# Wenlin-Chen/ADKF-IFT

Measured on AMD Instinct MI355X. Metric: meta-tasks/sec (N_support=128, d=256), higher is better.
Workload: dtype f32

## Files before the change

### adkf_ift_amd/_lib.py

```python
from __future__ import annotations

import ctypes as C
import os

_HERE = os.path.dirname(os.path.abspath(__file__))
LIB_PATH = os.path.join(_HERE, "libadkf_gp.so")
if os.environ.get("ADKF_LIB"):
    LIB_PATH = os.environ["ADKF_LIB"]

KERNEL_RBF = 0
KERNEL_MATERN52 = 1
IGNORE_GRAD_CORRECTION = 1
IGNORE_DIRECT_GRAD = 2
INFO_OUTER_BASE = 100000
PM_LATENT = 1
PM_MAXIMIZE = 2
PM_SCORE_MEAN = 4
POOL_TOPK_MAX = 64
TS_SAMPLES_MAX = 64
TS_FEATURES_MAX = 4096

ERRORS = {-1: "bad argument", -2: "unsupported size (see adkf_max_points)", -3: "workspace too small",
          -4: "HIP launch failed"}


class Batch(C.Structure):
    _fields_ = [("T", C.c_int32), ("ns_max", C.c_int32), ("nq_max", C.c_int32), ("d", C.c_int32),
                ("kernel", C.c_int32), ("flags", C.c_int32),
                ("n_s", C.c_void_p), ("n_q", C.c_void_p), ("Z_s", C.c_void_p), ("y_s", C.c_void_p),
                ("Z_q", C.c_void_p), ("y_q", C.c_void_p), ("priors", C.c_void_p)]


class MsgEt(C.Structure):
    _fields_ = [("src", C.c_void_p), ("tgt", C.c_void_p), ("W", C.c_void_p), ("bias", C.c_void_p), ("dW", C.c_void_p),
                ("db", C.c_void_p), ("E", C.c_int32)]


class FitOptions(C.Structure):
    _fields_ = [("max_evals", C.c_int32), ("exact_evals", C.c_int32), ("gtol", C.c_float), ("ftol", C.c_float),
                ("ev_start", C.c_void_p), ("ev_stop", C.c_void_p)]


_lib = None

SIGNATURES = {
    "adkf_version": (C.c_char_p, []),
    "adkf_last_hip_error": (C.c_char_p, []),
    "adkf_max_points": (C.c_int, []),
    "adkf_path_info": (C.c_int, [C.c_int32, C.c_int32]),
    "adkf_workspace_bytes": (C.c_size_t, [C.c_int32] * 4),
    "adkf_median_lengthscale": (C.c_int, [C.POINTER(Batch), C.c_void_p, C.c_void_p, C.c_size_t, C.c_void_p]),
    "adkf_init_params": (C.c_int, [C.POINTER(Batch), C.c_int32, C.c_int32, C.c_void_p, C.c_void_p, C.c_void_p,
                                   C.c_void_p, C.c_size_t, C.c_void_p]),
    "adkf_mll_value_grad": (C.c_int, [C.POINTER(Batch), C.c_void_p, C.c_void_p, C.c_void_p, C.c_void_p, C.c_void_p,
                                      C.c_void_p, C.c_size_t, C.c_void_p]),
    "adkf_fit": (C.c_int, [C.POINTER(Batch), C.c_void_p, C.POINTER(FitOptions), C.c_void_p, C.c_void_p, C.c_void_p,
                           C.c_void_p, C.c_void_p, C.c_size_t, C.c_void_p]),
    "adkf_predict": (C.c_int, [C.POINTER(Batch), C.c_void_p, C.c_void_p, C.c_void_p, C.c_void_p, C.c_void_p,
                               C.c_void_p, C.c_size_t, C.c_void_p]),
    "adkf_predict_marginal": (C.c_int, [C.POINTER(Batch), C.c_void_p, C.c_int32, C.c_void_p, C.c_void_p, C.c_int64, C.c_void_p,
                                        C.c_void_p, C.c_void_p, C.c_void_p, C.c_void_p, C.c_void_p, C.c_size_t, C.c_void_p]),
    "adkf_predict_marginal_ard": (C.c_int, [C.POINTER(Batch), C.c_void_p, C.c_int32, C.c_void_p, C.c_void_p, C.c_int64, C.c_void_p,
                                            C.c_void_p, C.c_void_p, C.c_void_p, C.c_void_p, C.c_void_p, C.c_size_t, C.c_void_p]),
    "adkf_predict_pool_scratch_bytes": (C.c_size_t, [C.c_int32, C.c_int32]),
    "adkf_predict_pool": (C.c_int, [C.POINTER(Batch), C.c_void_p, C.c_int32, C.c_void_p, C.c_int64, C.c_void_p, C.c_void_p, C.c_void_p,
                                    C.c_void_p, C.c_void_p, C.c_void_p, C.c_int32, C.c_void_p, C.c_void_p, C.c_void_p, C.c_void_p,
                                    C.c_size_t, C.c_void_p, C.c_size_t, C.c_void_p]),
    "adkf_thompson_pool_scratch_bytes": (C.c_size_t, [C.c_int32] * 4),
    "adkf_thompson_pool": (C.c_int, [C.POINTER(Batch), C.c_void_p, C.c_int32, C.c_void_p, C.c_int64, C.c_void_p, C.c_void_p, C.c_int32,
                                     C.c_void_p, C.c_void_p, C.c_int32, C.c_void_p, C.c_void_p, C.c_void_p, C.c_void_p, C.c_void_p,
                                     C.c_void_p, C.c_void_p, C.c_size_t, C.c_void_p, C.c_size_t, C.c_void_p]),
    "adkf_thompson_pool_ard": (C.c_int, [C.POINTER(Batch), C.c_void_p, C.c_int32, C.c_void_p, C.c_int64, C.c_void_p, C.c_void_p, C.c_int32,
                                         C.c_void_p, C.c_void_p, C.c_int32, C.c_void_p, C.c_void_p, C.c_void_p, C.c_void_p, C.c_void_p,
                                         C.c_void_p, C.c_void_p, C.c_size_t, C.c_void_p, C.c_size_t, C.c_void_p]),
    "adkf_outer_nll_value_grad": (C.c_int, [C.POINTER(Batch), C.c_void_p, C.c_void_p, C.c_void_p, C.c_void_p,
                                            C.c_void_p, C.c_void_p, C.c_void_p, C.c_size_t, C.c_void_p]),
    "adkf_ift_hypergrad": (C.c_int, [C.POINTER(Batch), C.c_void_p, C.c_int32, C.c_void_p, C.c_void_p, C.c_void_p,
                                     C.c_void_p, C.c_void_p, C.c_void_p, C.c_void_p, C.c_void_p, C.c_size_t,
                                     C.c_void_p]),
    "adkf_check_info": (C.c_int, [C.c_void_p, C.c_int32, C.c_void_p]),
    "adkf_workspace_bytes_ard": (C.c_size_t, [C.c_int32] * 4),
    "adkf_msg_forward": (C.c_int, [C.c_void_p, C.c_void_p, C.c_int32, C.c_int32, C.c_int32, C.c_int32, C.c_void_p, C.c_void_p]),
# ... 61 lines not shown
```

### adkf_ift_amd/csrc/adkf_gp.hip

```cpp
#include <hip/hip_runtime.h>
#include <algorithm>
#include <cstdio>
#include <cstdlib>

#include "../../include/adkf_gp.h"
#include "ard.h"
#include "pna.h"
#include "readout.h"
#include "block.h"
#include "outer_step.h"
#include "refine64.h"
#include "hyper.h"
#include "large_fused.h"
#include "gemm_x3.h"
#include "dense_x3.h"
#include "predict_stream.h"
#include "thompson_stream.h"

using namespace adkf;

namespace {

constexpr int MAX_POINTS = 4096;
constexpr int REG_POINTS = 128;

inline size_t align_up(size_t x) { return (x + 255) & ~size_t(255); }

inline int grid_for(int T, int tiles) { return ((T + 7) / 8) * 8 * tiles; }
inline int ceil_div(int a, int b) { return (a + b - 1) / b; }

inline int tiles_of(int M, int N) { return ceil_div(M, GT) * ceil_div(N, GT); }

template <class P> struct use_x3 : std::false_type {};
template <> struct use_x3<ProbDistMulti> : std::true_type {};
bool x3_enabled() {
    static const bool v = [] { const char* e = getenv("ADKF_X3"); return !(e && e[0] == '0'); }();
    return v;
}

inline bool x3_for(int d) { return x3_enabled() && d >= GK; }

template <class P>
void launch_gemm(const P& p, int T, int M, int N, hipStream_t st, bool x3 = false) {
    const int tm = ceil_div(M, GT), tn = ceil_div(N, GT);
    if constexpr (use_x3<P>::value) {
        if (x3 && x3_enabled()) { k_bgemm3<P, GT, 256><<<((T + 7) / 8) * 8 * tm * tn, 256, 0, st>>>(p, T, tm, tn); return; }
    }
    k_bgemm<P, GT><<<((T + 7) / 8) * 8 * tm * tn, 256, 0, st>>>(p, T, tm, tn);
}

// ... 370 lines not shown
        k_lg_resid<<<dim3(ceil_div(nq, 4), a.T), 256, 0, st>>>(a);
        LgMat m = lg_mat(w, a.S, a.tv.nq_ld, a.tv.n_q, nullptr, a.T);
        lg_sweep(m, st);
        LgMatvecArgs mv{m, a.vecs + (size_t)V_R * a.tv.vld, (size_t)NVEC * a.tv.vld, a.vecs + (size_t)V_E * a.tv.vld, (size_t)NVEC * a.tv.vld, -1.f};
        k_lg_matvec<<<dim3(ceil_div(nq, 4), a.T), 256, 0, st>>>(mv);
        const int tn = ceil_div(nq, GT);
        k_lg_negate<<<grid_for(a.T, tn * tn), 256, 0, st>>>(m, tn);
        LgColsumArgs cs{a.C, a.tv.ns_ld, (size_t)a.tv.nq_ld * a.tv.ns_ld, a.tv.n_q, a.tv.nq_ld, a.tv.n_s, a.tv.ns_ld,
                        a.vecs + (size_t)V_E * a.tv.vld, (size_t)NVEC * a.tv.vld, a.vecs + (size_t)V_CTE * a.tv.vld, (size_t)NVEC * a.tv.vld};
        k_lg_colsum<<<dim3(ceil_div(a.tv.ns_ld, 64), a.T), 1024, 0, st>>>(cs);
        LgOuterFin fin{a, w.lg_logdet, w.lg_info, w.lg_pext};
        k_lg_outer_fin<<<a.T, 64, 0, st>>>(fin);
        LAUNCH_OK();
        return 0;
    }
    if (nq <= 16) k_outer_factor<16, 256><<<grid_for(a.T, 1), 256, 0, st>>>(a);
    else if (nq <= 32) k_outer_factor<32, 256><<<grid_for(a.T, 1), 256, 0, st>>>(a);
    else if (nq <= 64) k_outer_factor<64, 256><<<grid_for(a.T, 1), 256, 0, st>>>(a);
    else k_outer_factor<128, 512><<<grid_for(a.T, 1), 512, 0, st>>>(a);
    LAUNCH_OK();
    return 0;
}


InnerArgs inner_args(const adkf_batch_t* b, const Workspace& w, float* phi, int32_t* info) {
    InnerArgs a{};
    a.D2ss = w.D2ss; a.y_s = b->y_s; a.n_s = b->n_s; a.phi = phi; a.priors = b->priors;
    a.Ainv = w.Ainv; a.vecs = w.vecs; a.scal = w.scal; a.info = info;
    a.T = b->T; a.ld = b->ns_max; a.vld = w.vld; a.kind = b->kernel;
    a.max_evals = 0; a.exact_evals = 0; a.gtol = 0.f; a.ftol = 0.f;
    return a;
}

int outer_pipeline(const adkf_batch_t* b, const Workspace& w, const float* phi, int flags, bool with_hessian, float* f_out,
                   float* dZ_s, float* dZ_q, float* g_phi_out, float* v_out, float* H_out, int32_t* info, hipStream_t st) {
    const int T = b->T, ns = b->ns_max, nq = b->nq_max, d = b->d;
    int rc = stage_dist(b, w, true, st);
    if (rc) return rc;
    const bool reuse_inner = (b->flags & ADKF_BATCH_REUSE_INNER) != 0;
    if (!reuse_inner) {
        InnerArgs ia = inner_args(b, w, const_cast<float*>(phi), info);
        rc = launch_inner(ia, w, st);
        if (rc) return rc;
    }
    TaskView tv = make_tv(b, w, true);
    const int tms = ceil_div(ns, GT), tmq = ceil_div(nq, GT);
    const float dirscale = (flags & ADKF_IGNORE_DIRECT_GRAD) ? 0.f : 1.f;
    const float corrscale = (with_hessian && !(flags & ADKF_IGNORE_GRAD_CORRECTION)) ? 1.f : 0.f;
    if (use_fused_outer(ns, nq)) {
        HyperArgs ha{tv, w.Ainv, w.D2ss, w.D2qs, w.D2qq, b->y_s, b->y_q, b->priors, w.Wss, w.Wqs, w.Wqq, w.P, w.OC, w.S, w.vecs, w.scal, f_out, info,
                     g_phi_out, v_out, H_out, T, reuse_inner ? 1 : 0, with_hessian ? 1 : 0, flags, dirscale, corrscale, refine32_threshold()};
        const bool full = ns == HY_N && nq == HY_N && !b->n_s && !b->n_q && tv.vec;
        const bool rbf = b->kernel == ADKF_KERNEL_RBF;
        if (full && rbf) k_hyper<true, 0><<<grid_for(T, 1), HY_NT, HY_LDS_BYTES, st>>>(ha);
        else if (full) k_hyper<true, 1><<<grid_for(T, 1), HY_NT, HY_LDS_BYTES, st>>>(ha);
        else if (rbf) k_hyper<false, 0><<<grid_for(T, 1), HY_NT, HY_LDS_BYTES, st>>>(ha);
        else k_hyper<false, 1><<<grid_for(T, 1), HY_NT, HY_LDS_BYTES, st>>>(ha);
    } else {
    launch_alpha_refine(tv, b, w, st);
    if (with_hessian) {
        ProbP pp; pp.tv = tv; pp.Ainv = w.Ainv; pp.D2ss = w.D2ss; pp.P = w.P;
        launch_gemm(pp, T, ns, ns, st);
        HessArgs ha{tv, w.Ainv, w.P, w.D2ss, b->y_s, b->priors, w.scal, w.vecs, T};
        if (ns > REG_POINTS) {
            k_lg_hess_mv<<<dim3(ceil_div(ns, 4), T), 256, 0, st>>>(ha);
            LgMat am = lg_mat(w, w.Ainv, ns, b->n_s, nullptr, T);
// ... 5 lines not shown
        } else {
            k_hess<<<grid_for(T, 1), SMALL_NT, 0, st>>>(ha);
        }
    }
    launch_c(tv, b, w, st);
    ProbS ps; ps.tv = tv; ps.C = w.C; ps.D2qs = w.D2qs; ps.D2qq = w.D2qq; ps.S = w.S;
    launch_gemm(ps, T, nq, nq, st);
    OuterArgs oa{tv, w.C, w.S, b->y_s, b->y_q, w.vecs, w.scal, f_out, info, T, reuse_inner ? 1 : 0};
    rc = launch_outer_factor(oa, w, nq, st);
    if (rc) return rc;
    ProbOC po; po.tv = tv; po.Sinv = w.S; po.C = w.C; po.D2qs = w.D2qs; po.OC = w.OC; po.Wqs = w.Wqs; po.part = w.part_oc; po.ntiles = w.nt_oc; po.dirscale = dirscale;
    launch_gemm(po, T, nq, ns, st);
    ProbMA pm; pm.tv = tv; pm.C = w.C; pm.OC = w.OC; pm.D2ss = w.D2ss; pm.Wss = w.Wss; pm.part = w.part_ma; pm.ntiles = w.nt_ma; pm.dirscale = dirscale;
    launch_gemm(pm, T, ns, ns, st);
    SolveArgs sa{tv, w.scal, w.vecs, w.part_oc, w.part_ma, w.nt_oc, w.nt_ma, flags, g_phi_out, v_out, H_out, T, with_hessian ? 1 : 0};
    WqqArgs wq{tv, w.S, w.D2qq, w.Wqq, w.scal, dirscale, T, 0, sa};
    if (nq > REG_POINTS) {
        LgWqq lw{wq, w.lg_part, tmq * tmq, tmq};
        k_lg_wqq<<<grid_for(T, tmq * tmq), 256, 0, st>>>(lw);
        k_lg_wqq_fin<<<T, 64, 0, st>>>(lw);
        k_solve_v<<<T, 64, 0, st>>>(sa);
    } else {
        wq.do_solve = 1;
        k_wqq<<<grid_for(T, 1), SMALL_NT, 0, st>>>(wq);
    }
    if (corrscale != 0.f) {
        ProbMixed px; px.tv = tv; px.Ainv = w.Ainv; px.P = w.P; px.D2ss = w.D2ss; px.Wss = w.Wss; px.corrscale = corrscale;
        launch_gemm(px, T, ns, ns, st);
    }
    }
    if (dZ_s || dZ_q) {
        if (dZ_s && b->n_s) hipMemsetAsync(dZ_s, 0, (size_t)T * ns * d * sizeof(float), st);
        if (dZ_q && b->n_q) hipMemsetAsync(dZ_q, 0, (size_t)T * nq * d * sizeof(float), st);
        ProbDZ<false> pzs; pzs.tv = tv; pzs.Wss = w.Wss; pzs.Wqs = w.Wqs; pzs.Wqq = w.Wqq; pzs.Zs = b->Z_s; pzs.Zq = b->Z_q; pzs.dZ = dZ_s; pzs.d = d;
        ProbDZ<true> pzq; pzq.tv = tv; pzq.Wss = w.Wss; pzq.Wqs = w.Wqs; pzq.Wqq = w.Wqq; pzq.Zs = b->Z_s; pzq.Zq = b->Z_q; pzq.dZ = dZ_q; pzq.d = d;
        if (dZ_s) launch_gemm(pzs, T, ns, d, st, x3_for(d));
        if (dZ_q) launch_gemm(pzq, T, nq, d, st, x3_for(d));
    }
    if (w.w64) {
        size_t lds_bytes;
        const Refine64Args ra = refine_args(tv, b, w, with_hessian, 2, f_out, info, nullptr, nullptr, nullptr, lds_bytes);
        Cot64Args ca{tv, b->Z_s, b->Z_q, dZ_s, dZ_q, d, w.vecs, w.scal, w.w64, w.w64_stride, r64_threshold(), T,
                     with_hessian ? 1 : 0, flags, dirscale, corrscale, g_phi_out, v_out, H_out, lds_bytes ? 1 : 0};
        k_tail64<<<T, R64_NT, lds_bytes, st>>>(ra, ca);
    }
    LAUNCH_OK();
    return 0;
}


struct ArdWs {
    float *mu, *ell, *Zt_s, *Zt_q, *G, *Gd_s, *Gd_q, *Gdot, *phi3, *pri3, *f3, *g3, *g3o, *S1, *gt, *coldot;
    float *c, *ut2, *wn, *Ddot, *Wdot, *adot, *S2;
    ArdFitState* fst; float *x, *g, *p, *xe, *ge, *S, *Y, *fe; int32_t* info3;
    ArdCgState* cst; float *cx, *cr, *cp, *cHp, *gout; int32_t* n_eff;
    size_t bytes;
};

ArdWs carve_ard(void* base, size_t off0, int T, int ns, int nq, int d) {
    ArdWs a;
    size_t off = off0;
    auto take = [&](size_t nfloat) { float* p = base ? reinterpret_cast<float*>(static_cast<char*>(base) + off) : nullptr; off += align_up((nfloat ? nfloat : 1) * sizeof(float)); return p; };
    const size_t Tz = (size_t)T, h = 2 + (size_t)d;
    a.mu = take(Tz * d); a.ell = take(Tz * d);
    a.Zt_s = take(Tz * ns * d); a.Zt_q = take(Tz * nq * d);
    a.G = take(Tz * ns * d); a.Gd_s = take(Tz * ns * d); a.Gd_q = take(Tz * nq * d); a.Gdot = take(Tz * ns * d);
    a.phi3 = take(Tz * 3); a.pri3 = take(Tz * 4); a.f3 = take(Tz); a.g3 = take(Tz * 3); a.g3o = take(Tz * 3);
    a.S1 = take(Tz * d); a.gt = take(Tz * h); a.coldot = take(Tz * d);
    a.c = take(Tz * d); a.ut2 = take(Tz * 2); a.wn = take(Tz * ns);
    a.Ddot = take(Tz * ns * ns); a.Wdot = take(Tz * ns * ns); a.adot = take(Tz * ns); a.S2 = take(Tz * d);
// ... 135 lines not shown

int predict_core(const adkf_batch_t* b, const Workspace& w, float* mean, float* var, float* cov, int32_t* info, hipStream_t st) {
    TaskView tv = make_tv(b, w, true);
    const int T = b->T;
    launch_alpha_refine(tv, b, w, st);
    launch_c(tv, b, w, st);
    launch_refine(tv, b, w, false, 1, nullptr, info, st);
    PredArgs pa{tv, w.C, w.D2qs, b->y_s, mean, var, w.scal, T};
    k_predict<<<grid_for(T, 1), 256, 0, st>>>(pa);
    if (cov) {
        hipMemsetAsync(cov, 0, (size_t)T * b->nq_max * b->nq_max * sizeof(float), st);
        ProbS ps; ps.tv = tv; ps.C = w.C; ps.D2qs = w.D2qs; ps.D2qq = w.D2qq; ps.S = cov;
        launch_gemm(ps, T, b->nq_max, b->nq_max, st);
    }
    LAUNCH_OK();
    return 0;
}

int ard_outer(ArdCtx& c, const float* phi, int flags, float* f_out, int32_t* info, bool want_grads) {
    hipStream_t st = c.st;
    int rc;
    if (!(c.b->flags & ADKF_BATCH_REUSE_INNER)) {
        rc = ard_eval(c, phi, c.a.fe, c.a.ge, c.a.info3);
        if (rc) return rc;
        hipMemcpyAsync(info, c.a.info3, sizeof(int32_t) * (size_t)c.T, hipMemcpyDeviceToDevice, st);
    } else {
        hipMemsetAsync(info, 0, sizeof(int32_t) * (size_t)c.T, st);
    }
    k_ard_scale<<<dim3(ceil_div(c.nq, 4), c.T), 256, 0, st>>>(c.v, c.b->Z_q, c.a.Zt_q, c.b->n_q, c.nq);
    rc = stage_dist(&c.bt, c.w, true, st, 2 | 4);
    if (rc) return rc;
    if (!want_grads) return 0;
    adkf_batch_t bq = c.bt;
    bq.flags = ADKF_BATCH_REUSE_DIST | ADKF_BATCH_REUSE_INNER;
    int32_t* info_o = c.a.info3;
    rc = outer_pipeline(&bq, c.w, c.a.phi3, flags & ADKF_IGNORE_DIRECT_GRAD, false, f_out, c.a.Gd_s, c.a.Gd_q, c.a.g3o, nullptr, nullptr, info_o, st);
    if (rc) return rc;
    ArdColdot cd{c.a.Zt_s, c.a.Gd_s, c.b->n_s, c.ns, c.a.Zt_q, c.a.Gd_q, c.b->n_q, c.nq, c.a.coldot, c.d};
    k_ard_coldot<<<dim3(ceil_div(c.d, 64), c.T), 256, 0, st>>>(cd);
    ArdGout go{c.v, phi, c.a.coldot, c.a.g3o, c.a.gout};
    k_ard_gout<<<dim3(ceil_div(c.d, 256), c.T), 256, 0, st>>>(go);
    LAUNCH_OK();
    return 0;
}

__global__ void k_merge_info(const int32_t* extra, int32_t* info, int T) {
    const int t = blockIdx.x * blockDim.x + threadIdx.x;
    if (t < T && info[t] == 0 && extra[t] != 0) info[t] = extra[t];
}

int ard_ift(const adkf_batch_t* b, const float* phi, int flags, bool with_hessian, int cg_maxiter, float cg_tol, float* f_out,
            float* dZ_s, float* dZ_q, float* g_phi_out, float* v_out, int32_t* cg_iters, int32_t* info, void* ws, size_t ws_bytes,
            hipStream_t st) {
    ArdCtx c;
    int rc = ard_setup(b, ws, ws_bytes, st, c);
    if (rc) return rc;
    if (b->flags & ADKF_BATCH_REUSE_INNER) k_ard_params<<<dim3(ceil_div(c.d, 256), c.T), 256, 0, st>>>(c.v, phi);
    rc = ard_outer(c, phi, flags, f_out, info, true);
    if (rc) return rc;
    k_merge_info<<<ceil_div(c.T, 64), 64, 0, st>>>(c.a.info3, info, c.T);
    const size_t hb = sizeof(float) * (size_t)c.T * c.h;
    if (g_phi_out) hipMemcpyAsync(g_phi_out, c.a.gout, hb, hipMemcpyDeviceToDevice, st);
    const bool correct = with_hessian && !(flags & ADKF_IGNORE_GRAD_CORRECTION);
    if (correct) {
        ArdCg cg{c.T, c.h, cg_tol, c.a.cst, c.a.gout, c.a.cx, c.a.cr, c.a.cp, c.a.cHp, b->n_s, c.ns, c.a.n_eff};
        k_ard_cg_begin<<<c.T, 256, 0, st>>>(cg);
        FitPoll poll(true, cg_maxiter, c.a.info3, st);
// ... 532 lines not shown
                           const int64_t* excl_off, float* paths, int64_t* sel_idx, float* sel_val, int32_t* info, void* ws, size_t ws_bytes,
                           void* scratch, size_t scratch_bytes, void* stream) {
    return thompson_pool(true, b, phi, flags, X, rows, omega, phase, m, w, eps, S, excl_idx, excl_off, paths, sel_idx, sel_val, info, ws,
                         ws_bytes, scratch, scratch_bytes, stream);
}

int adkf_outer_nll_value_grad(const adkf_batch_t* b, const float* phi, float* f_out, float* g_phi, float* dZ_s,
                              float* dZ_q, int32_t* info, void* ws, size_t ws_bytes, void* stream) {
    int rc = check_batch(b, true);
    if (rc) return rc;
    if (!phi || !f_out || !info || !ws || !b->y_s || !b->y_q || !b->priors) return ADKF_E_BADARG;
    if (is_ard(b))
        return ard_ift(b, phi, 0, false, 0, 0.f, f_out, dZ_s, dZ_q, g_phi, nullptr, nullptr, info, ws, ws_bytes, static_cast<hipStream_t>(stream));
    Workspace w = carve_for(b, ws);
    if (ws_bytes < w.bytes) return ADKF_E_WORKSPACE;
    return outer_pipeline(b, w, phi, 0, false, f_out, dZ_s, dZ_q, g_phi, nullptr, nullptr, info, static_cast<hipStream_t>(stream));
}

int adkf_ift_hypergrad(const adkf_batch_t* b, const float* phi, int32_t flags, float* f_out, float* dZ_s, float* dZ_q,
                       float* g_phi_out, float* v, float* H, int32_t* info, void* ws, size_t ws_bytes, void* stream) {
    int rc = check_batch(b, true);
    if (rc) return rc;
    if (!phi || !f_out || !dZ_s || !dZ_q || !info || !ws || !b->y_s || !b->y_q || !b->priors) return ADKF_E_BADARG;
    if (is_ard(b)) {
        if (H) return ADKF_E_BADARG;
        return ard_ift(b, phi, flags, true, ADKF_CG_DEFAULT_MAXITER, ADKF_CG_DEFAULT_TOL, f_out, dZ_s, dZ_q, g_phi_out, v, nullptr, info,
                       ws, ws_bytes, static_cast<hipStream_t>(stream));
    }
    Workspace w = carve_for(b, ws);
    if (ws_bytes < w.bytes) return ADKF_E_WORKSPACE;
    return outer_pipeline(b, w, phi, flags, true, f_out, dZ_s, dZ_q, g_phi_out, v, H, info, static_cast<hipStream_t>(stream));
}

int adkf_double_path_tasks(const adkf_batch_t* b, int32_t* flagged, void* ws, size_t ws_bytes, void* stream) {
    int rc = check_batch(b, true);
    if (rc) return rc;
    if (!flagged || !ws || is_ard(b)) return ADKF_E_BADARG;
    Workspace w = carve_for(b, ws);
    if (ws_bytes < w.bytes) return ADKF_E_WORKSPACE;
    (void)hipGetLastError();
    k_double_path_tasks<<<ceil_div(b->T, 256), 256, 0, static_cast<hipStream_t>(stream)>>>(w.scal, b->ns_max, b->nq_max, w.w64 ? r64_threshold() : INFINITY, b->T, flagged);
    LAUNCH_OK();
    return 0;
}

size_t adkf_workspace_bytes_ard(int32_t T, int32_t ns_max, int32_t nq_max, int32_t d) {
    if (T <= 0 || ns_max <= 0 || nq_max < 0 || d <= 0) return 0;
    return carve_ard(nullptr, carve(nullptr, T, ns_max, nq_max, d).bytes, T, ns_max, nq_max, d).bytes;
}

int adkf_ift_hypergrad_cg(const adkf_batch_t* b, const float* phi, int32_t flags, int32_t cg_maxiter, float cg_tol, float* f_out,
                          float* dZ_s, float* dZ_q, float* g_phi_out, float* v, int32_t* cg_iters, int32_t* info, void* ws,
                          size_t ws_bytes, void* stream) {
    int rc = check_batch(b, true);
    if (rc) return rc;
    if (!is_ard(b) || cg_maxiter < 1 || !(cg_tol > 0.f)) return ADKF_E_BADARG;
    if (!phi || !f_out || !dZ_s || !dZ_q || !info || !ws || !b->y_s || !b->y_q || !b->priors) return ADKF_E_BADARG;
    return ard_ift(b, phi, flags, true, cg_maxiter, cg_tol, f_out, dZ_s, dZ_q, g_phi_out, v, cg_iters, info, ws, ws_bytes,
                   static_cast<hipStream_t>(stream));
}

namespace {
long msg_table(MsgArgs& m, const adkf_msg_et_t* ets, int n_et, bool backward) {
    long e_all = 0;
    int splits = 0;
    for (int q = 0; q < n_et; ++q) {
// ... 400 lines not shown
```

### adkf_ift_amd/csrc/cpu/adkf_gp_cpu.cpp

```cpp
#include <algorithm>
#include <cmath>
#include <cstdint>
#include <cstring>
#include <limits>
#include <vector>

#include "adkf_gp.h"

namespace {

using Mat = std::vector<double>;
constexpr double NOISE_LB = 1e-4, LOG_2PI = 1.8378770664093453, SQRT5 = 2.23606797749979;

inline double softplus(double x) { return x > 30.0 ? x : std::log1p(std::exp(x)); }
inline double sigmoid(double x) { return 1.0 / (1.0 + std::exp(-x)); }
inline double inv_softplus(double y) { return y > 30.0 ? y : y + std::log(-std::expm1(-y)); }

inline void kappa(int kind, double u, double& k0, double& k1, double& k2) {
    if (kind == ADKF_KERNEL_RBF) { k0 = std::exp(-0.5 * u); k1 = -0.5 * k0; k2 = 0.25 * k0; return; }
    const double r = std::sqrt(u), e = std::exp(-SQRT5 * r);
    k0 = (1.0 + SQRT5 * r + (5.0 / 3.0) * u) * e; k1 = -(5.0 / 6.0) * (1.0 + SQRT5 * r) * e; k2 = (25.0 / 12.0) * e;
}

template <class F>
// ... 379 lines not shown
    void reset_H() { for (int i = 0; i < 3; ++i) for (int j = 0; j < 3; ++j) Hi[i][j] = i == j; first = true; }
    bool direction() {
        for (int i = 0; i < 3; ++i) p[i] = -(Hi[i][0] * g[0] + Hi[i][1] * g[1] + Hi[i][2] * g[2]);
        gp = g[0] * p[0] + g[1] * p[1] + g[2] * p[2];
        if (!(gp < 0.0)) { reset_H(); for (int i = 0; i < 3; ++i) p[i] = -g[i]; gp = -(g[0] * g[0] + g[1] * g[1] + g[2] * g[2]); if (!(gp < 0.0)) return false; }
        step = first ? std::min(1.0, 1.0 / (std::fabs(g[0]) + std::fabs(g[1]) + std::fabs(g[2]))) : 1.0;
        step = std::min(step, 16.0 / std::max(std::max(std::fabs(p[0]), std::fabs(p[1])), std::max(std::fabs(p[2]), 1e-30)));
        bt = 0;
        return true;
    }
    void accept(const double* xn, double fn, const double* gn) {
        double s[3], yv[3];
        for (int i = 0; i < 3; ++i) { s[i] = xn[i] - x[i]; yv[i] = gn[i] - g[i]; x[i] = xn[i]; g[i] = gn[i]; }
        f = fn;
        const double sy = s[0] * yv[0] + s[1] * yv[1] + s[2] * yv[2], yy = yv[0] * yv[0] + yv[1] * yv[1] + yv[2] * yv[2], ss = s[0] * s[0] + s[1] * s[1] + s[2] * s[2];
        if (sy > 1e-10 * std::sqrt(ss * yy) && yy > 0.0) {
            if (first) { const double sc = sy / yy; for (int i = 0; i < 3; ++i) for (int j = 0; j < 3; ++j) Hi[i][j] = i == j ? sc : 0.0; first = false; }
            const double rho = 1.0 / sy;
            double Hy[3];
            for (int i = 0; i < 3; ++i) Hy[i] = Hi[i][0] * yv[0] + Hi[i][1] * yv[1] + Hi[i][2] * yv[2];
            const double yHy = yv[0] * Hy[0] + yv[1] * Hy[1] + yv[2] * Hy[2];
            for (int i = 0; i < 3; ++i) for (int j = 0; j < 3; ++j) Hi[i][j] += -rho * (s[i] * Hy[j] + Hy[i] * s[j]) + rho * (rho * yHy + 1.0) * s[i] * s[j];
        }
    }
};

}

extern "C" {

const char* adkf_version(void) { return "adkf_gp_cpu 0.1 (float64 inside, OpenMP over tasks)"; }
const char* adkf_last_hip_error(void) { return "no HIP in the CPU twin"; }
int adkf_max_points(void) { return 1 << 20; }
size_t adkf_workspace_bytes(int32_t, int32_t, int32_t, int32_t) { return 0; }

int adkf_median_lengthscale(const adkf_batch_t* b, float* l0, void*, size_t, void*) {
    if (int rc = check(b, false)) return rc;
    if (!l0) return ADKF_E_BADARG;
#pragma omp parallel for schedule(dynamic)
    for (int t = 0; t < b->T; ++t) {
        const int n = ns_of(b, t);
        const float* Z = b->Z_s + (size_t)t * b->ns_max * b->d;
        l0[t] = n > 1 ? (float)median_l0(sqdist(Z, n, Z, n, b->d), n) : 0.f;
    }
    return 0;
}

int adkf_init_params(const adkf_batch_t* b, int32_t numeric, int32_t use_ls_prior, float* phi, float* priors, float* l0, void*, size_t, void*) {
    if (int rc = check(b, false)) return rc;
    if (!phi || !priors) return ADKF_E_BADARG;
#pragma omp parallel for schedule(dynamic)
    for (int t = 0; t < b->T; ++t) {
        const int n = ns_of(b, t);
        const float* Z = b->Z_s + (size_t)t * b->ns_max * b->d;
        const float l = n > 1 ? (float)median_l0(sqdist(Z, n, Z, n, b->d), n) : 0.f;
        if (l0) l0[t] = l;
        const double scale = 0.25, mode = numeric ? 0.01 : 0.1;
        phi[t * 3 + 0] = (float)inv_softplus(mode - NOISE_LB); phi[t * 3 + 1] = 0.f; phi[t * 3 + 2] = (float)inv_softplus((double)l);
        priors[t * 4 + 0] = (float)(std::log(mode) + scale * scale); priors[t * 4 + 1] = (float)scale;
        priors[t * 4 + 2] = use_ls_prior ? (float)(std::log((double)l) + scale * scale) : 0.f; priors[t * 4 + 3] = use_ls_prior ? (float)scale : -1.f;
    }
    return 0;
}

int adkf_mll_value_grad(const adkf_batch_t* b, const float* phi, float* f_in, float* g_phi, float* dZ_s, int32_t* info, void*, size_t, void*) {
    if (int rc = check(b, false)) return rc;
// ... 302 lines not shown
```

### adkf_ift_amd/gp_ops.py

```python
from __future__ import annotations

import ctypes as C
from dataclasses import dataclass
from typing import Optional, Tuple

import torch

from . import _lib
from ._lib import KERNEL_MATERN52, KERNEL_RBF, Batch, FitOptions

KERNELS = {"rbf": KERNEL_RBF, "RBF": KERNEL_RBF, "matern": KERNEL_MATERN52}
REUSE_DIST = 1
REUSE_INNER = 2
LG_UNFUSED = 16
LG_FUSED = 32
DEFER_REFINE = 8
ARD = 4


def kernel_id(kernel) -> int:
    if isinstance(kernel, int):
        return kernel
    if kernel not in KERNELS:
        raise ValueError("[ERROR] the kernel '" + str(kernel) + "' is not supported!")
    return KERNELS[kernel]


FTOL_DEFAULT = 2.22e-9


def _ptr(t: Optional[torch.Tensor]):
    return None if t is None else C.c_void_p(t.data_ptr())


def _f32(t: Optional[torch.Tensor], name: str) -> Optional[torch.Tensor]:
    if t is None:
        return None
    if not t.is_cuda:
        raise RuntimeError(f"{name} must live on the GPU: the GP path has no CPU fallback")
    if t.dtype != torch.float32:
        t = t.float()
    return t.contiguous()


@dataclass
class GPBatch:

    Z_s: torch.Tensor
# ... 390 lines not shown
    info = _new(b, b.T, dtype=torch.int32)
    sb = int(lib.adkf_thompson_pool_scratch_bytes(b.T, b.ns, S, m))
    scratch = torch.empty(sb, dtype=torch.uint8, device=b.device)
    ws, nb = b.workspace()
    cb = b.c_struct()
    entry = "adkf_" + name
    _lib.check(getattr(lib, entry)(C.byref(cb), _ptr(phi), _lib.PM_MAXIMIZE if maximize else 0, _ptr(X), rows, _ptr(omega), _ptr(phase),
                                   m, _ptr(w), _ptr(eps), S, _ptr(excl_idx), _ptr(excl_off), _ptr(paths), _ptr(sel_idx), _ptr(sel_val),
                                   _ptr(info), _ptr(ws), nb, _ptr(scratch), sb, _stream(b.device)), entry)
    return dict(sel_idx=sel_idx, sel_val=sel_val, paths=paths, info=info, w=w, eps=eps)


def thompson_pool(b: GPBatch, phi: torch.Tensor, X: torch.Tensor, *, omega: torch.Tensor, phase: torch.Tensor, n_samples: int,
                  generator: Optional[torch.Generator] = None, w: Optional[torch.Tensor] = None, eps: Optional[torch.Tensor] = None,
                  maximize: bool = False, exclude=None, want_paths: bool = False):
    return _thompson_pool("thompson_pool", b, phi, X, omega, phase, n_samples, generator, w, eps, maximize, exclude, want_paths)


def thompson_pool_ard(b: GPBatch, phi: torch.Tensor, X: torch.Tensor, *, omega: torch.Tensor, phase: torch.Tensor, n_samples: int,
                      generator: Optional[torch.Generator] = None, w: Optional[torch.Tensor] = None, eps: Optional[torch.Tensor] = None,
                      maximize: bool = False, exclude=None, want_paths: bool = False):
    return _thompson_pool("thompson_pool_ard", b, phi, X, omega, phase, n_samples, generator, w, eps, maximize, exclude, want_paths)


def double_path_tasks(b: GPBatch) -> torch.Tensor:
    lib = _lib.load()
    flagged = _new(b, b.T, dtype=torch.int32)
    ws, nb = b.workspace()
    cb = b.c_struct()
    _lib.check(lib.adkf_double_path_tasks(C.byref(cb), _ptr(flagged), _ptr(ws), nb, _stream(b.device)), "adkf_double_path_tasks")
    return flagged


def outer_nll_value_grad(b: GPBatch, phi: torch.Tensor, want_grads=True):
    lib = _lib.load()
    phi = b.check_phi(phi)
    f = _new(b, b.T)
    g = _new(b, b.T, b.h) if want_grads else None
    dZs = _new(b, b.T, b.ns, b.d) if want_grads else None
    dZq = _new(b, b.T, b.nq, b.d) if want_grads else None
    info = _new(b, b.T, dtype=torch.int32)
    ws, nb = b.workspace()
    cb = b.c_struct()
    _lib.check(lib.adkf_outer_nll_value_grad(C.byref(cb), _ptr(phi), _ptr(f), _ptr(g), _ptr(dZs), _ptr(dZq), _ptr(info),
                                             _ptr(ws), nb, _stream(b.device)), "adkf_outer_nll_value_grad")
    return f, g, dZs, dZq, info


def ift_hypergrad(b: GPBatch, phi: torch.Tensor, ignore_grad_correction=False, ignore_direct_grad=False, out_dZ=None,
                  cg_maxiter: Optional[int] = None, cg_tol: float = 1e-6):
    lib = _lib.load()
    phi = b.check_phi(phi)
    flags = (_lib.IGNORE_GRAD_CORRECTION if ignore_grad_correction else 0) | (_lib.IGNORE_DIRECT_GRAD if ignore_direct_grad else 0)
    if out_dZ is not None:
        dZ_s, dZ_q = out_dZ
        assert dZ_s.is_contiguous() and dZ_q.is_contiguous() and dZ_s.dtype == torch.float32 and dZ_q.dtype == torch.float32
        assert dZ_s.shape == b.Z_s.shape and dZ_q.shape == b.Z_q.shape
    else:
        dZ_s, dZ_q = _new(b, b.T, b.ns, b.d), _new(b, b.T, b.nq, b.d)
    ws, nb = b.workspace()
    cb = b.c_struct()
    if b.ard:
        out = dict(f_out=_new(b, b.T), dZ_s=dZ_s, dZ_q=dZ_q, g_phi=_new(b, b.T, b.h), v=_new(b, b.T, b.h), H=None,
                   info=_new(b, b.T, dtype=torch.int32), cg_iters=_new(b, b.T, dtype=torch.int32))
        _lib.check(lib.adkf_ift_hypergrad_cg(C.byref(cb), _ptr(phi), flags, int(cg_maxiter or 48), float(cg_tol), _ptr(out["f_out"]),
                                             _ptr(dZ_s), _ptr(dZ_q), _ptr(out["g_phi"]), _ptr(out["v"]), _ptr(out["cg_iters"]),
# ... 10 lines not shown
```

### include/adkf_gp.h

```cpp
#ifndef ADKF_GP_H
#define ADKF_GP_H

#include <stddef.h>
#include <stdint.h>

#ifdef __cplusplus
extern "C" {
#endif

#define ADKF_KERNEL_RBF 0
#define ADKF_KERNEL_MATERN52 1

#define ADKF_E_BADARG (-1)
#define ADKF_E_SIZE (-2)
#define ADKF_E_WORKSPACE (-3)
#define ADKF_E_LAUNCH (-4)

#define ADKF_INFO_OUTER_BASE 100000

#define ADKF_BATCH_REUSE_DIST 1
#define ADKF_BATCH_REUSE_INNER 2

#define ADKF_BATCH_DEFER_REFINE 8

#define ADKF_BATCH_LG_UNFUSED 16
#define ADKF_BATCH_LG_FUSED 32

#define ADKF_BATCH_ARD 4
#define ADKF_CG_DEFAULT_MAXITER 48
#define ADKF_CG_DEFAULT_TOL 1e-6f
#define ADKF_INFO_CG_BASE 200000

#define ADKF_IGNORE_GRAD_CORRECTION 1
#define ADKF_IGNORE_DIRECT_GRAD 2

typedef struct adkf_batch {
    int32_t T;
    int32_t ns_max;
    int32_t nq_max;
    int32_t d;
    int32_t kernel;
    int32_t flags;
    const int32_t* n_s;
    const int32_t* n_q;
    const float* Z_s;
    const float* y_s;
    const float* Z_q;
    const float* y_q;
    const float* priors;
} adkf_batch_t;

typedef struct adkf_fit_options {
    int32_t max_evals;
    int32_t exact_evals;
    float gtol;
    float ftol;
    void* ev_start;
    void* ev_stop;
} adkf_fit_options_t;

const char* adkf_version(void);

const char* adkf_last_hip_error(void);

#define ADKF_PATH_FUSED_OUTER 1
#define ADKF_PATH_BLOCKED 2
#define ADKF_PATH_BLOCKED_FUSED 4
#define ADKF_PATH_R64_REGION 8
#define ADKF_PATH_R64_LDS 16
int adkf_path_info(int32_t ns_max, int32_t nq_max);

int adkf_max_points(void);

size_t adkf_workspace_bytes(int32_t T, int32_t ns_max, int32_t nq_max, int32_t d);

int adkf_median_lengthscale(const adkf_batch_t* b, float* l0, void* ws, size_t ws_bytes, void* stream);

int adkf_init_params(const adkf_batch_t* b, int32_t use_numeric_labels, int32_t use_lengthscale_prior,
                     float* phi, float* priors, float* l0, void* ws, size_t ws_bytes, void* stream);

int adkf_mll_value_grad(const adkf_batch_t* b, const float* phi, float* f_in, float* g_phi, float* dZ_s,
                        int32_t* info, void* ws, size_t ws_bytes, void* stream);

int adkf_fit(const adkf_batch_t* b, float* phi, const adkf_fit_options_t* opt, float* f_final, float* gnorm,
             int32_t* n_evals, int32_t* info, void* ws, size_t ws_bytes, void* stream);

int adkf_predict(const adkf_batch_t* b, const float* phi, float* mean, float* var, float* cov, int32_t* info,
                 void* ws, size_t ws_bytes, void* stream);

#define ADKF_PM_LATENT 1
#define ADKF_PM_MAXIMIZE 2
int adkf_predict_marginal(const adkf_batch_t* b, const float* phi, int32_t flags, const float* Zq, const int64_t* q_off, int64_t rows, const float* best_f, float* mean, float* var, float* ei, int32_t* info, void* ws, size_t ws_bytes, void* stream);

int adkf_predict_marginal_ard(const adkf_batch_t* b, const float* phi, int32_t flags, const float* Zq, const int64_t* q_off, int64_t rows, const float* best_f, float* mean, float* var, float* ei, int32_t* info, void* ws, size_t ws_bytes, void* stream);

#define ADKF_PM_SCORE_MEAN 4
#define ADKF_POOL_TOPK_MAX 64
size_t adkf_predict_pool_scratch_bytes(int32_t T, int32_t k);
int adkf_predict_pool(const adkf_batch_t* b, const float* phi, int32_t flags, const float* X, int64_t rows, const float* best_f, const int64_t* excl_idx, const int64_t* excl_off, float* mean, float* var, float* ei, int32_t k, int64_t* top_idx, float* top_val, int32_t* info, void* ws, size_t ws_bytes, void* scratch, size_t scratch_bytes, void* stream);

#define ADKF_TS_SAMPLES_MAX 64
#define ADKF_TS_FEATURES_MAX 4096
size_t adkf_thompson_pool_scratch_bytes(int32_t T, int32_t ns_max, int32_t S, int32_t m);
// ... 97 lines not shown
```

Baseline: 284,900.

## Fuse support and query dZ gradient GEMMs into one LDS-staged MFMA slab kernel

Adds a dedicated kernel that computes both dZ_s and dZ_q in one launch for fixed 128-point support/query tasks with d a multiple of 64. Each block handles one task and side, double-buffers scaled W tiles and Z tiles in LDS, runs fp32 MFMA, and folds the row-sum diagonal term into the epilogue. This replaces two generic GEMM launches and the separate output memsets, cutting launch overhead and extra passes over W. It needs a large dynamic-LDS opt-in and falls back to the old path for other shapes, ARD, or when a new DZ_TILED flag is set (as the IFT path now does).

```diff
diff --git a/adkf_ift_amd/_lib.py b/adkf_ift_amd/_lib.py
--- a/adkf_ift_amd/_lib.py
+++ b/adkf_ift_amd/_lib.py
@@ -48,6 +48,7 @@
     "adkf_last_hip_error": (C.c_char_p, []),
     "adkf_max_points": (C.c_int, []),
     "adkf_path_info": (C.c_int, [C.c_int32, C.c_int32]),
+    "adkf_dz_one_launch": (C.c_int, [C.POINTER(Batch)]),
     "adkf_workspace_bytes": (C.c_size_t, [C.c_int32] * 4),
     "adkf_median_lengthscale": (C.c_int, [C.POINTER(Batch), C.c_void_p, C.c_void_p, C.c_size_t, C.c_void_p]),
     "adkf_init_params": (C.c_int, [C.POINTER(Batch), C.c_int32, C.c_int32, C.c_void_p, C.c_void_p, C.c_void_p,
diff --git a/adkf_ift_amd/csrc/adkf_gp.hip b/adkf_ift_amd/csrc/adkf_gp.hip
--- a/adkf_ift_amd/csrc/adkf_gp.hip
+++ b/adkf_ift_amd/csrc/adkf_gp.hip
@@ -16,6 +16,7 @@
 #include "dense_x3.h"
 #include "predict_stream.h"
 #include "thompson_stream.h"
+#include "dz.h"
 
 using namespace adkf;
 
@@ -452,6 +453,18 @@
     return a;
 }
 
+bool dz_slab_optin() {
+    static const bool ok = hipFuncSetAttribute(reinterpret_cast<const void*>(&k_dz_slab), hipFuncAttributeMaxDynamicSharedMemorySize, (int)DZ_LDS_BYTES) == hipSuccess;
+    if (!ok) (void)hipGetLastError();
+    return ok;
+}
+
+bool use_dz_slab(const adkf_batch_t* b, bool vec, bool both) {
+    if (!both || (b->flags & (ADKF_BATCH_DZ_TILED | ADKF_BATCH_ARD))) return false;
+    if (b->ns_max != DZ_N || b->nq_max != DZ_N || b->n_s || b->n_q || !b->Z_q || (b->d % 64) != 0 || !vec) return false;
+    return dz_slab_optin();
+}
+
 int outer_pipeline(const adkf_batch_t* b, const Workspace& w, const float* phi, int flags, bool with_hessian, float* f_out,
                    float* dZ_s, float* dZ_q, float* g_phi_out, float* v_out, float* H_out, int32_t* info, hipStream_t st) {
     const int T = b->T, ns = b->ns_max, nq = b->nq_max, d = b->d;
@@ -523,10 +536,15 @@
     if (dZ_s || dZ_q) {
         if (dZ_s && b->n_s) hipMemsetAsync(dZ_s, 0, (size_t)T * ns * d * sizeof(float), st);
         if (dZ_q && b->n_q) hipMemsetAsync(dZ_q, 0, (size_t)T * nq * d * sizeof(float), st);
-        ProbDZ<false> pzs; pzs.tv = tv; pzs.Wss = w.Wss; pzs.Wqs = w.Wqs; pzs.Wqq = w.Wqq; pzs.Zs = b->Z_s; pzs.Zq = b->Z_q; pzs.dZ = dZ_s; pzs.d = d;
-        ProbDZ<true> pzq; pzq.tv = tv; pzq.Wss = w.Wss; pzq.Wqs = w.Wqs; pzq.Wqq = w.Wqq; pzq.Zs = b->Z_s; pzq.Zq = b->Z_q; pzq.dZ = dZ_q; pzq.d = d;
-        if (dZ_s) launch_gemm(pzs, T, ns, d, st, x3_for(d));
-        if (dZ_q) launch_gemm(pzq, T, nq, d, st, x3_for(d));
+        if (use_dz_slab(b, tv.vec, dZ_s && dZ_q)) {
+            DzArgs da{w.Wss, w.Wqs, w.Wqq, b->Z_s, b->Z_q, dZ_s, dZ_q, d, T};
+            k_dz_slab<<<grid_for(T, 2), DZ_NT, DZ_LDS_BYTES, st>>>(da);
+        } else {
+            ProbDZ<false> pzs; pzs.tv = tv; pzs.Wss = w.Wss; pzs.Wqs = w.Wqs; pzs.Wqq = w.Wqq; pzs.Zs = b->Z_s; pzs.Zq = b->Z_q; pzs.dZ = dZ_s; pzs.d = d;
+            ProbDZ<true> pzq; pzq.tv = tv; pzq.Wss = w.Wss; pzq.Wqs = w.Wqs; pzq.Wqq = w.Wqq; pzq.Zs = b->Z_s; pzq.Zq = b->Z_q; pzq.dZ = dZ_q; pzq.d = d;
+            if (dZ_s) launch_gemm(pzs, T, ns, d, st, x3_for(d));
+            if (dZ_q) launch_gemm(pzq, T, nq, d, st, x3_for(d));
+        }
     }
     if (w.w64) {
         size_t lds_bytes;
@@ -728,7 +746,7 @@
     if (rc) return rc;
     if (!want_grads) return 0;
     adkf_batch_t bq = c.bt;
-    bq.flags = ADKF_BATCH_REUSE_DIST | ADKF_BATCH_REUSE_INNER;
+    bq.flags = ADKF_BATCH_REUSE_DIST | ADKF_BATCH_REUSE_INNER | ADKF_BATCH_DZ_TILED;
     int32_t* info_o = c.a.info3;
     rc = outer_pipeline(&bq, c.w, c.a.phi3, flags & ADKF_IGNORE_DIRECT_GRAD, false, f_out, c.a.Gd_s, c.a.Gd_q, c.a.g3o, nullptr, nullptr, info_o, st);
     if (rc) return rc;
@@ -1327,6 +1345,13 @@
     return outer_pipeline(b, w, phi, flags, true, f_out, dZ_s, dZ_q, g_phi_out, v, H, info, static_cast<hipStream_t>(stream));
 }
 
+int adkf_dz_one_launch(const adkf_batch_t* b) {
+    int rc = check_batch(b, true);
+    if (rc) return rc;
+    const Workspace w = carve(nullptr, b->T, b->ns_max, b->nq_max, b->d);
+    return use_dz_slab(b, vec_ok(b, w), true) ? 1 : 0;
+}
+
 int adkf_double_path_tasks(const adkf_batch_t* b, int32_t* flagged, void* ws, size_t ws_bytes, void* stream) {
     int rc = check_batch(b, true);
     if (rc) return rc;
diff --git a/adkf_ift_amd/csrc/cpu/adkf_gp_cpu.cpp b/adkf_ift_amd/csrc/cpu/adkf_gp_cpu.cpp
--- a/adkf_ift_amd/csrc/cpu/adkf_gp_cpu.cpp
+++ b/adkf_ift_amd/csrc/cpu/adkf_gp_cpu.cpp
@@ -435,6 +435,7 @@
 const char* adkf_version(void) { return "adkf_gp_cpu 0.1 (float64 inside, OpenMP over tasks)"; }
 const char* adkf_last_hip_error(void) { return "no HIP in the CPU twin"; }
 int adkf_max_points(void) { return 1 << 20; }
+int adkf_dz_one_launch(const adkf_batch_t* b) { if (int rc = check(b, true, true)) return rc; return 0; }
 size_t adkf_workspace_bytes(int32_t, int32_t, int32_t, int32_t) { return 0; }
 
 int adkf_median_lengthscale(const adkf_batch_t* b, float* l0, void*, size_t, void*) {
diff --git a/adkf_ift_amd/csrc/dz.h b/adkf_ift_amd/csrc/dz.h
--- /dev/null
+++ b/adkf_ift_amd/csrc/dz.h
@@ -0,0 +1,167 @@
+#pragma once
+#include "problems.h"
+
+namespace adkf {
+
+constexpr int DZ_N = 128;
+constexpr int DZ_NT = 512;
+constexpr int DZ_PW = 256;
+constexpr int DZ_LDZ = DZ_PW + 16;
+constexpr int DZ_A_FLOATS = DZ_N * LD_MN;
+constexpr int DZ_BUF_FLOATS = DZ_A_FLOATS + GK * DZ_LDZ;
+constexpr size_t DZ_LDS_BYTES = sizeof(float) * (2 * DZ_BUF_FLOATS + DZ_N);
+
+struct DzArgs {
+    const float *Wss, *Wqs, *Wqq;
+    const float *Zs, *Zq;
+    float *dZs, *dZq;
+    int d, T;
+};
+
+__global__ __launch_bounds__(DZ_NT) void k_dz_slab(DzArgs a) {
+    constexpr int N = DZ_N, NCH = 2 * N / GK, SEG = N / GK, MI = 4;
+    int task, slab;
+    if (!task_tile(a.T, 2, task, slab)) return;
+    extern __shared__ float4 dz_lds[];
+    float* const lds = reinterpret_cast<float*>(dz_lds);
+    float* const rowsum = lds + 2 * DZ_BUF_FLOATS;
+
+    const bool query = slab != 0;
+    const int d = a.d;
+    const float* const W0 = (query ? a.Wqs : a.Wss) + (size_t)task * N * N;
+    const float* const W1 = (query ? a.Wqq : a.Wqs) + (size_t)task * N * N;
+    const float f0 = query ? 2.f : 4.f, f1 = query ? 4.f : 2.f;
+    const float* const Zs = a.Zs + (size_t)task * N * d;
+    const float* const Zq = a.Zq + (size_t)task * N * d;
+    const float* const Zo = query ? Zq : Zs;
+    float* const out = (query ? a.dZq : a.dZs) + (size_t)task * N * d;
+
+    const int tid = threadIdx.x, lane = tid & 63, wv = tid >> 6;
+    const int wr = wv >> 2, wc = wv & 3;
+    const int fi = lane & 15, fk = lane >> 4;
+    const int zj = lane * 4, zk = wv;
+    const int ar = tid >> 3, ak = (tid & 7) * 4;
+    const int ti = (tid & 31) * 4, tk = tid >> 5;
+
+    for (int p0 = 0; p0 < d; p0 += DZ_PW) {
+        const int width = d - p0 < DZ_PW ? d - p0 : DZ_PW;
+        const bool zload = zj < width, mult = wc * 64 < width;
+        float4 qa[2], qz[4];
+
+        auto fetch = [&](int c) __attribute__((always_inline)) {
+            const int k0 = (c % SEG) * GK;
+            const float* const Zc = (c < SEG ? Zs : Zq) + (size_t)k0 * d + p0;
+            if (zload) {
+#pragma unroll
+                for (int ps = 0; ps < 4; ++ps) qz[ps] = ldq(Zc + (size_t)(zk + 8 * ps) * d + zj);
+            }
+            if (c < SEG || query) {
+                const float* const W = (c < SEG ? W0 : W1) + k0 + ak;
+#pragma unroll
+                for (int ps = 0; ps < 2; ++ps) qa[ps] = ldq(W + (size_t)(ar + 64 * ps) * N);
+            } else {
+#pragma unroll
+                for (int ps = 0; ps < 2; ++ps) qa[ps] = ldq(W1 + (size_t)(k0 + tk + 16 * ps) * N + ti);
+            }
+        };
+        auto stage = [&](int c) __attribute__((always_inline)) {
+            float* const As = lds + (c & 1) * DZ_BUF_FLOATS;
+            float* const Zb = As + DZ_A_FLOATS;
+            if (zload) {
+#pragma unroll
+                for (int ps = 0; ps < 4; ++ps) *reinterpret_cast<float4*>(Zb + (zk + 8 * ps) * DZ_LDZ + zj) = qz[ps];
+            }
+            const float f = c < SEG ? f0 : f1;
+#pragma unroll
+            for (int ps = 0; ps < 2; ++ps) {
+                float v[4];
+                unq(qa[ps], v);
+#pragma unroll
+                for (int x = 0; x < 4; ++x) v[x] *= f;
+                if (c < SEG || query) {
+#pragma unroll
+                    for (int x = 0; x < 4; ++x) As[(ar + 64 * ps) * LD_MN + ak + x] = v[x];
+                } else {
+#pragma unroll
+                    for (int x = 0; x < 4; ++x) As[(ti + x) * LD_MN + tk + 16 * ps] = v[x];
+                }
+            }
+        };
+
+        f32x4 acc[MI][MI];
+#pragma unroll
+        for (int i = 0; i < MI; ++i)
+#pragma unroll
+            for (int j = 0; j < MI; ++j) acc[i][j] = (f32x4){0.f, 0.f, 0.f, 0.f};
+        float sq[2] = {0.f, 0.f};
+
+        fetch(0);
+        stage(0);
+        __syncthreads();
+        auto multiply = [&](int c) __attribute__((always_inline)) {
+            const float* const As = lds + (c & 1) * DZ_BUF_FLOATS;
+            const float* const Zb = As + DZ_A_FLOATS;
+#pragma unroll
+            for (int ps = 0; ps < 2; ++ps)
+#pragma unroll
+                for (int x = 0; x < 4; ++x) sq[ps] += As[(ar + 64 * ps) * LD_MN + ak + x];
+            if (mult) {
+#pragma unroll
+                for (int s = 0; s < GK / 4; ++s) {
+                    float af[MI], bf[MI];
+#pragma unroll
+                    for (int i = 0; i < MI; ++i) af[i] = As[(wr * 64 + i * 16 + fi) * LD_MN + 4 * s + fk];
+#pragma unroll
+                    for (int j = 0; j < MI; ++j) bf[j] = Zb[(4 * s + fk) * DZ_LDZ + wc * 64 + j * 16 + fi];
+#pragma unroll
+                    for (int i = 0; i < MI; ++i)
+#pragma unroll
+                        for (int j = 0; j < MI; ++j)
+                            acc[i][j] = __builtin_amdgcn_mfma_f32_16x16x4f32(af[i], bf[j], acc[i][j], 0, 0, 0);
+                }
+            }
+        };
+#pragma unroll 1
+        for (int c = 0; c + 1 < NCH; ++c) {
+            fetch(c + 1);
+            __builtin_amdgcn_sched_barrier(0);
+            multiply(c);
+            stage(c + 1);
+            __syncthreads();
+        }
+        multiply(NCH - 1);
+
+#pragma unroll
+        for (int ps = 0; ps < 2; ++ps) {
+            float s = sq[ps];
+            s += dpp_f<DPP_XOR1>(s); s += dpp_f<DPP_XOR2>(s); s += dpp_f<DPP_HALF_MIRROR>(s);
+            if ((tid & 7) == 0) rowsum[ar + 64 * ps] = s;
+        }
+        __syncthreads();
+
+        if (mult) {
+#pragma unroll
+            for (int h = 0; h < MI; h += 2) {
+                float zv[2][MI][4];
+#pragma unroll
+                for (int i = 0; i < 2; ++i)
+#pragma unroll
+                    for (int j = 0; j < MI; ++j)
+#pragma unroll
+                        for (int r = 0; r < 4; ++r)
+                            zv[i][j][r] = Zo[(size_t)(wr * 64 + (h + i) * 16 + fk * 4 + r) * d + p0 + wc * 64 + j * 16 + fi];
+#pragma unroll
+                for (int i = 0; i < 2; ++i)
+#pragma unroll
+                    for (int j = 0; j < MI; ++j)
+#pragma unroll
+                        for (int r = 0; r < 4; ++r) {
+                            const int gi = wr * 64 + (h + i) * 16 + fk * 4 + r;
+                            out[(size_t)gi * d + p0 + wc * 64 + j * 16 + fi] = rowsum[gi] * zv[i][j][r] - acc[h + i][j][r];
+                        }
+            }
+        }
+    }
+}
+
+}
diff --git a/adkf_ift_amd/gp_ops.py b/adkf_ift_amd/gp_ops.py
--- a/adkf_ift_amd/gp_ops.py
+++ b/adkf_ift_amd/gp_ops.py
@@ -14,6 +14,7 @@
 REUSE_INNER = 2
 LG_UNFUSED = 16
 LG_FUSED = 32
+DZ_TILED = 64
 DEFER_REFINE = 8
 ARD = 4
 
@@ -470,6 +471,15 @@
     return flagged
 
 
+def dz_one_launch(b: GPBatch) -> bool:
+    lib = _lib.load()
+    cb = b.c_struct()
+    rc = lib.adkf_dz_one_launch(C.byref(cb))
+    if rc < 0:
+        _lib.check(rc, "adkf_dz_one_launch")
+    return rc == 1
+
+
 def outer_nll_value_grad(b: GPBatch, phi: torch.Tensor, want_grads=True):
     lib = _lib.load()
     phi = b.check_phi(phi)
diff --git a/include/adkf_gp.h b/include/adkf_gp.h
--- a/include/adkf_gp.h
+++ b/include/adkf_gp.h
@@ -25,6 +25,7 @@
 
 #define ADKF_BATCH_LG_UNFUSED 16
 #define ADKF_BATCH_LG_FUSED 32
+#define ADKF_BATCH_DZ_TILED 64
 
 #define ADKF_BATCH_ARD 4
 #define ADKF_CG_DEFAULT_MAXITER 48
@@ -69,6 +70,8 @@
 #define ADKF_PATH_R64_REGION 8
 #define ADKF_PATH_R64_LDS 16
 int adkf_path_info(int32_t ns_max, int32_t nq_max);
+
+int adkf_dz_one_launch(const adkf_batch_t* b);
 
 int adkf_max_points(void);
 
```

Measured after the change: 291,700 (median of 6 runs). 2.4% higher.
